# HenryHZY/VL-PET

Hardware: AMD Instinct MI355X
Metric: multitask samples/sec (BART-base, r=96) (higher is better)
Workload: dtype bf16

## Files before the change

### include/vlpet_hip.h

```cpp
#ifndef VLPET_HIP_H
#define VLPET_HIP_H
#include <stddef.h>
#include <stdint.h>

#ifdef __cplusplus
extern "C" {
#endif

#define VLPET_F32 0
#define VLPET_BF16 1

#define VLPET_E_SHAPE (-1)
#define VLPET_E_RANK (-2)
#define VLPET_E_ALIGN (-3)
#define VLPET_E_WORKSPACE (-4)
#define VLPET_E_NULL (-5)
#define VLPET_E_DTYPE (-6)
#define VLPET_E_ALIAS (-7)

#define VLPET_GATE_NONE 0
#define VLPET_GATE_MUL 1
#define VLPET_GATE_ADD 2

typedef void* vlpet_stream_t;

int vlpet_version(void);
const char* vlpet_error_string(int code);

int vlpet_rank_tiles(int r);

size_t vlpet_packed_bytes(int tiles, int d, int io_dtype);
int vlpet_pack_pair(const void* const* wd_heads, const void* const* bd_heads, int n_heads,
                    const void* wu, const void* bu, int r, int d, int tiles,
// ... 203 lines not shown
int vlpet_act_dropout_fwd(const void* x, void* out, uint8_t* keep_out, int64_t n, int act, float p, uint64_t seed,
                          int io_dtype, vlpet_stream_t stream);
int vlpet_act_dropout_bwd(const void* dy, const void* x, void* dx, int64_t n, int act, float p, uint64_t seed,
                          int io_dtype, vlpet_stream_t stream);
int vlpet_concat_dropout_fwd(const void* a, const void* v, void* x, int64_t B, int La, int Lv, int d, float p, uint64_t seed,
                             int io_dtype, vlpet_stream_t stream);
int vlpet_concat_dropout_bwd(const void* dx, void* da, void* dv, int64_t B, int La, int Lv, int d, float p, uint64_t seed,
                             int io_dtype, vlpet_stream_t stream);

int vlpet_ce_loss_fwd(const void* logits, const int64_t* labels, float* loss, float* lse, int64_t N, int V, int ld,
                      int io_dtype, vlpet_stream_t stream);
int vlpet_ce_loss_bwd(const void* logits, const int64_t* labels, const float* lse, const float* dloss, void* dlogits,
                      int64_t N, int V, int ld, int io_dtype, vlpet_stream_t stream);
int vlpet_ce_loss_fwd_checked(const void* logits, const int64_t* labels, float* loss, float* lse, unsigned int* bad_count,
                              int64_t N, int V, int ld, int io_dtype, vlpet_stream_t stream);

#define VLPET_ATTN_MAX_LEN 128
int vlpet_attn_fwd(const void* q, const void* k, const void* v, const uint8_t* key_mask, void* o, float* lse, uint8_t* keep_out,
                   int B, int H, int Lq, int Lk, int causal, float scale, float p, uint64_t seed, vlpet_stream_t stream);
int vlpet_attn_bwd(const void* q, const void* k, const void* v, const void* o, const void* dout, const float* lse,
                   const uint8_t* key_mask, void* dq, void* dk, void* dv, int B, int H, int Lq, int Lk, int causal,
                   float scale, float p, uint64_t seed, vlpet_stream_t stream);
int vlpet_attn_fwd_ld(const void* q, const void* k, const void* v, const uint8_t* key_mask, void* o, float* lse, uint8_t* keep_out,
                      int B, int H, int Lq, int Lk, int ld_q, int ld_kv, int causal, float scale, float p, uint64_t seed,
                      vlpet_stream_t stream);
int vlpet_attn_bwd_ld(const void* q, const void* k, const void* v, const void* o, const void* dout, const float* lse,
                      const uint8_t* key_mask, void* dq, void* dk, void* dv, int B, int H, int Lq, int Lk, int ld_q, int ld_kv,
                      int causal, float scale, float p, uint64_t seed, vlpet_stream_t stream);
int vlpet_attn_fwd_bias(const void* q, const void* k, const void* v, const uint8_t* key_mask, const float* bias, void* o,
                        float* lse, uint8_t* keep_out, int B, int H, int Lq, int Lk, int ld_q, int ld_kv, int causal,
// ... 112 lines not shown
```

### vl-pet_amd/_lib.py

```python
from __future__ import annotations

import ctypes
import os
from ctypes import c_char_p, c_float, c_int, c_int64, c_size_t, c_uint64, c_void_p

_HERE = os.path.dirname(os.path.abspath(__file__))
LIB_PATH = os.environ.get("VLPET_LIB") or os.path.join(_HERE, "lib", "libvlpet_hip.so")

VLPET_F32 = 0
VLPET_BF16 = 1
GATE_NONE, GATE_MUL, GATE_ADD = 0, 1, 2

_lib = None

SIGNATURES = {
    "vlpet_version": (c_int, []),
    "vlpet_error_string": (c_char_p, [c_int]),
    "vlpet_rank_tiles": (c_int, [c_int]),
    "vlpet_packed_bytes": (c_size_t, [c_int, c_int, c_int]),
    "vlpet_pack_pair": (c_int, [c_void_p, c_void_p, c_int, c_void_p, c_void_p, c_int, c_int, c_int, c_int, c_int,
                                c_void_p, c_void_p]),
    "vlpet_pack_pairs": (c_int, [c_int, c_void_p, c_void_p, c_int, c_void_p, c_void_p, c_int, c_int, c_int, c_int, c_int,
                                 c_void_p, c_void_p]),
    "vlpet_adapter_gate_fwd": (c_int, [c_void_p, c_void_p, c_void_p, c_void_p, c_void_p, c_int64, c_int, c_int,
# ... 99 lines not shown
    "vlpet_attn_bwd": (c_int, [c_void_p] * 10 + [c_int] * 5 + [c_float, c_float, c_uint64, c_void_p]),
    "vlpet_attn_fwd_ld": (c_int, [c_void_p] * 7 + [c_int] * 7 + [c_float, c_float, c_uint64, c_void_p]),
    "vlpet_attn_bwd_ld": (c_int, [c_void_p] * 10 + [c_int] * 7 + [c_float, c_float, c_uint64, c_void_p]),
    "vlpet_attn_fwd_bias": (c_int, [c_void_p] * 8 + [c_int] * 7 + [c_float, c_float, c_uint64, c_void_p]),
    "vlpet_attn_bwd_bias": (c_int, [c_void_p] * 12 + [c_int] * 7 + [c_float, c_float, c_uint64, c_void_p]),
    "vlpet_concat_dropout_fwd": (c_int, [c_void_p] * 3 + [c_int64, c_int, c_int, c_int, c_float, c_uint64, c_int, c_void_p]),
    "vlpet_concat_dropout_bwd": (c_int, [c_void_p] * 3 + [c_int64, c_int, c_int, c_int, c_float, c_uint64, c_int, c_void_p]),
    "vlpet_attn_fwd_kv": (c_int, [c_void_p] * 8 + [c_int] * 8 + [c_float, c_float, c_uint64, c_void_p]),
    "vlpet_attn_bwd_kv": (c_int, [c_void_p] * 12 + [c_int] * 8 + [c_float, c_float, c_uint64, c_void_p]),
    "vlpet_attn_long_fwd": (c_int, [c_void_p] * 7 + [c_int] * 8 + [c_float, c_void_p]),
    "vlpet_attn_long_fwd_train": (c_int, [c_void_p] * 8 + [c_int] * 8 + [c_float, c_float, c_uint64, c_void_p]),
    "vlpet_attn_long_bwd": (c_int, [c_void_p] * 12 + [c_int] * 8 + [c_float, c_float, c_uint64, c_void_p, c_void_p]),
    "vlpet_ce_loss_fwd": (c_int, [c_void_p] * 4 + [c_int64, c_int, c_int, c_int, c_void_p]),
    "vlpet_ce_loss_fwd_checked": (c_int, [c_void_p] * 5 + [c_int64, c_int, c_int, c_int, c_void_p]),
    "vlpet_ce_loss_bwd": (c_int, [c_void_p] * 5 + [c_int64, c_int, c_int, c_int, c_void_p]),
    "vlpet_act_dropout_fwd": (c_int, [c_void_p] * 3 + [c_int64, c_int, c_float, c_uint64, c_int, c_void_p]),
    "vlpet_act_dropout_bwd": (c_int, [c_void_p] * 3 + [c_int64, c_int, c_float, c_uint64, c_int, c_void_p]),
    "vlpet_attn_decode": (c_int, [c_void_p, c_int64, c_void_p, c_void_p, c_int64, c_int64, c_int64, c_int64, c_void_p, c_void_p,
                                  c_int64, c_int, c_void_p, c_int64, c_void_p, c_int64, c_void_p, c_int64, c_int, c_int, c_int,
                                  c_int, c_float, c_int, c_void_p]),
    "vlpet_greedy_pick": (c_int, [c_void_p, c_int64, c_int, c_void_p, c_int64, c_int, c_void_p, c_void_p, c_int, c_int, c_int,
                                  c_int, c_int, c_int, c_void_p]),
    "vlpet_attn_decode_beam": (c_int, [c_void_p, c_int64, c_void_p, c_void_p, c_int64, c_int64, c_int64, c_int64, c_void_p,
                                       c_void_p, c_int64, c_int, c_void_p, c_int64, c_void_p, c_int64, c_void_p, c_int64, c_int,
                                       c_int, c_int, c_int, c_float, c_int, c_void_p, c_int64, c_int, c_void_p]),
    "vlpet_beam_rows": (c_int, [c_void_p, c_int64, c_int, c_void_p, c_int64, c_int, c_int, c_int, c_int, c_int, c_int, c_int, c_int,
                                c_void_p, c_void_p, c_void_p, c_int, c_void_p]),
    "vlpet_beam_advance": (c_int, [c_void_p, c_void_p, c_void_p, c_int, c_int, c_int, c_int, c_void_p, c_void_p, c_void_p, c_int64,
                                   c_void_p, c_void_p, c_int64, c_void_p, c_void_p, c_void_p, c_void_p, c_int64, c_void_p,
                                   c_void_p, c_void_p, c_int, c_int, c_int, c_float, c_int, c_void_p]),
# ... 47 lines not shown
```

### vl-pet_amd/csrc/api.hip

```cpp
#include <atomic>
#include "../../include/vlpet_hip.h"
#include "common.h"
#include "kernels.h"
#include <cmath>
#include <stdlib.h>
#include <stdio.h>
#include <vector>

#define VLPET_VERSION 670
#define VLPET_VERSION_R3 300
#define VLPET_VERSION_R2 221

static inline bool aligned16(const void* p) { return (reinterpret_cast<uintptr_t>(p) & 15) == 0; }
static inline size_t align256(size_t v) { return (v + 255) / 256 * 256; }
static inline int herr(hipError_t e) { return e == hipSuccess ? 0 : (int)e; }

extern "C" int vlpet_version(void) { return VLPET_VERSION; }
extern "C" int vlpet_debug_build(void) { return VLPET_IS_DEBUG_BUILD; }

__global__ __launch_bounds__(64) void hold_cus_kernel(unsigned* release, unsigned long long ticks) {
    extern __shared__ __attribute__((aligned(16))) uint8_t hold_smem[];
    typedef __attribute__((address_space(1))) unsigned gu32;
    if (threadIdx.x == 0) {
        hold_smem[0] = 1;
// ... 11 lines not shown
    hipLaunchKernelGGL(hold_cus_kernel, dim3((unsigned)workgroups), dim3(64), (size_t)lds_bytes, (hipStream_t)stream,
                       reinterpret_cast<unsigned*>(release_flag), (unsigned long long)max_ms * 100000ull);
    return herr(hipGetLastError());
}

extern "C" const char* vlpet_error_string(int code) {
    switch (code) {
        case 0: return "success";
        case VLPET_E_SHAPE: return "bad shape (need M > 0, d % 64 == 0, r > 0)";
        case VLPET_E_RANK: return "unsupported bottleneck rank (max 192) or tile count";
        case VLPET_E_ALIGN: return "pointer not 16-byte aligned";
        case VLPET_E_WORKSPACE: return "workspace too small";
        case VLPET_E_NULL: return "required pointer is NULL";
        case VLPET_E_DTYPE: return "unsupported dtype";
        case VLPET_E_ALIAS: return "output overlaps an input";
        default: return code > 0 ? hipGetErrorString((hipError_t)code) : "unknown error";
    }
}

extern "C" int vlpet_rank_tiles(int r) {
    if (r <= 0) return VLPET_E_SHAPE;
    if (r <= 32) return 1;
    if (r <= 96) return 3;
    if (r <= 192) return 6;
    return VLPET_E_RANK;
}

static inline bool tiles_ok(int t) { return t == 1 || t == 3 || t == 6; }
static inline bool dtype_ok(int t) { return t == VLPET_F32 || t == VLPET_BF16; }

// ... 1306 lines not shown
    return vlpet_ce_loss_fwd_checked(logits, labels, loss, lse, nullptr, N, V, ld, io_dtype, stream);
}

extern "C" int vlpet_ce_loss_bwd(const void* logits, const int64_t* labels, const float* lse, const float* dloss, void* dlogits,
                                 int64_t N, int V, int ld, int io_dtype, vlpet_stream_t stream) {
    int rc = ce_common(N, V, ld, io_dtype);
    if (rc) return rc;
    if (!logits || !labels || !lse || !dloss || !dlogits) return VLPET_E_NULL;
    if (!aligned16(logits) || !aligned16(dlogits)) return VLPET_E_ALIGN;
    CeArgs a{};
    a.logits = logits; a.labels = labels; a.loss = nullptr; a.lse = const_cast<float*>(lse); a.dloss = dloss; a.dlogits = dlogits;
    a.N = N; a.V = V; a.ld = ld;
    return herr(launch_ce(a, true, io_dtype == VLPET_F32, (hipStream_t)stream));
}

static int act_common(int64_t n, int act, float p, int io_dtype) {
    if (n <= 0 || (n & 7) != 0) return VLPET_E_SHAPE;
    if (act != VLPET_ACT_GELU && act != VLPET_ACT_GELU_NEW && act != VLPET_ACT_RELU) return VLPET_E_SHAPE;
    if (!(p >= 0.0f && p < 1.0f)) return VLPET_E_SHAPE;
    if (io_dtype != VLPET_F32 && io_dtype != VLPET_BF16) return VLPET_E_DTYPE;
    return 0;
}

extern "C" int vlpet_act_dropout_fwd(const void* x, void* out, uint8_t* keep_out, int64_t n, int act, float p, uint64_t seed,
                                     int io_dtype, vlpet_stream_t stream) {
    int rc = act_common(n, act, p, io_dtype);
    if (rc) return rc;
    if (!x || !out) return VLPET_E_NULL;
    if (!aligned16(x) || !aligned16(out)) return VLPET_E_ALIGN;
    ActDropArgs a{};
// ... 261 lines not shown
```

### vl-pet_amd/csrc/celoss.hip

```cpp
#include "common.h"
#include "kernels.h"
#include "vec8.h"

#define CE_THREADS 256

__device__ __forceinline__ float wave_max(float v) {
#pragma unroll
    for (int o = 32; o > 0; o >>= 1) v = fmaxf(v, __shfl_xor(v, o));
    return v;
}
__device__ __forceinline__ float wave_sum(float v) {
#pragma unroll
    for (int o = 32; o > 0; o >>= 1) v += __shfl_xor(v, o);
    return v;
}

template <typename IO>
__global__ __launch_bounds__(CE_THREADS) void ce_fwd_kernel(CeArgs a) {
    __shared__ float sm[CE_THREADS / 64], ss[CE_THREADS / 64];
    const int64_t n = blockIdx.x;
    const int64_t lab = a.labels[n];
    if (lab < 0 || lab >= a.V) {
        if (threadIdx.x == 0) {
            a.loss[n] = 0.f; a.lse[n] = 0.f;
            if (a.bad != nullptr && lab != -100) atomicAdd(a.bad, 1u);
        }
        return;
    }
    const IO* row = reinterpret_cast<const IO*>(a.logits) + n * (int64_t)a.ld;
    const int groups = (a.V + 7) >> 3;
    float m = -INFINITY, s = 0.f;
    for (int g = threadIdx.x; g < groups; g += CE_THREADS) {
        Vec8<IO> x;
        x.load(row, g);
        float v[8], cm = -INFINITY;
#pragma unroll
        for (int j = 0; j < 8; ++j) {
            v[j] = (8 * g + j < a.V) ? x.get(j) : -INFINITY;
            cm = fmaxf(cm, v[j]);
        }
        const float mn = fmaxf(m, cm);
        float acc = 0.f;
#pragma unroll
        for (int j = 0; j < 8; ++j) acc += __expf(v[j] - mn);
        s = s * __expf(m - mn) + acc;
        m = mn;
    }
    const int wave = threadIdx.x >> 6, lane = threadIdx.x & 63;
    const float wm = wave_max(m);
    const float wsum = wave_sum(m == -INFINITY ? 0.f : s * __expf(m - wm));
    if (lane == 0) { sm[wave] = wm; ss[wave] = wsum; }
    __syncthreads();
    if (threadIdx.x == 0) {
        float M = sm[0];
#pragma unroll
        for (int w = 1; w < CE_THREADS / 64; ++w) M = fmaxf(M, sm[w]);
        float S = 0.f;
#pragma unroll
        for (int w = 0; w < CE_THREADS / 64; ++w) S += ss[w] * __expf(sm[w] - M);
        const float lse = M + __logf(S);
        a.lse[n] = lse;
        a.loss[n] = lse - (float)row[lab];
    }
}

template <typename IO>
__global__ __launch_bounds__(CE_THREADS) void ce_bwd_kernel(CeArgs a) {
    const int64_t n = blockIdx.x;
    const int64_t lab = a.labels[n];
    const bool live = lab >= 0 && lab < a.V;
    const float g = live ? a.dloss[n] : 0.f;
    const IO* row = reinterpret_cast<const IO*>(a.logits) + n * (int64_t)a.ld;
    IO* out = reinterpret_cast<IO*>(a.dlogits) + n * (int64_t)a.ld;
    const int groups = a.ld >> 3;
    if (g == 0.f) {
// ... 6 lines not shown
    const float lse = a.lse[n];
    for (int gi = threadIdx.x; gi < groups; gi += CE_THREADS) {
        Vec8<IO> x, o;
        x.load(row, gi);
#pragma unroll
        for (int j = 0; j < 8; ++j) {
            const int v = 8 * gi + j;
            float p = v < a.V ? __expf(x.get(j) - lse) : 0.f;
            if (v == (int)lab) p -= 1.0f;
            o.set(j, g * p);
        }
        o.store(out, gi);
    }
}

hipError_t launch_ce(const CeArgs& a, bool bwd, int io_fp32, hipStream_t stream) {
    if (a.N <= 0) return hipSuccess;
    const dim3 grid((unsigned)a.N), blk(CE_THREADS);
    if (bwd) {
        if (io_fp32) hipLaunchKernelGGL(ce_bwd_kernel<float>, grid, blk, 0, stream, a);
        else hipLaunchKernelGGL(ce_bwd_kernel<__bf16>, grid, blk, 0, stream, a);
    } else {
        if (io_fp32) hipLaunchKernelGGL(ce_fwd_kernel<float>, grid, blk, 0, stream, a);
        else hipLaunchKernelGGL(ce_fwd_kernel<__bf16>, grid, blk, 0, stream, a);
    }
    return hipGetLastError();
}
```

### vl-pet_amd/csrc/kernels.h

```cpp
#pragma once
#include <cstdlib>
#include <hip/hip_runtime.h>
#include <stdint.h>
#include "rng.h"
#include "tuning.h"

#define VLPET_MAX_HEADS 16

struct PackArgs {
    const void* wd[VLPET_MAX_HEADS];
    const void* bd[VLPET_MAX_HEADS];
    const void* wu;
    const void* bu;
    int n_heads, rows_per_head;
    int r, d, RT;
    int src_bf16;
    int n_packs;
    uint8_t* out;
};
hipError_t launch_pack_pair(const PackArgs& a, int NS, hipStream_t stream);
#define VLPET_PACK_BATCH 8
struct PackBatch { PackArgs p[VLPET_PACK_BATCH]; int n; };
hipError_t launch_pack_pairs(const PackBatch& b, int NS, hipStream_t stream);

// ... 341 lines not shown
hipError_t launch_cat_dropout(const void* a, const void* v, void* x, int64_t B, int La, int Lv, int d, uint32_t thr, float keep_scale,
                              uint64_t seed, const uint64_t* seed_ctr, bool bwd, int io_fp32, hipStream_t stream);

struct CeArgs {
    const void* logits;
    const int64_t* labels;
    float* loss;
    float* lse;
    const float* dloss;
    void* dlogits;
    int64_t N;
    int V, ld;
    unsigned int* bad;
};
hipError_t launch_ce(const CeArgs& a, bool bwd, int io_fp32, hipStream_t stream);

struct AttnArgs {
    const __bf16* q; const __bf16* k; const __bf16* v;
    __bf16* o;
    float* lse;
    const __bf16* dout;
    __bf16* dq; __bf16* dk; __bf16* dv;
    const uint8_t* key_mask;
    const float* bias;
    const float* bias_t;
    uint8_t* keep_out;
    int B, H, Lq, Lk, causal;
    int ld_q, ld_kv;
    int ld_v;
    float scale;
// ... 49 lines not shown
```

### vl-pet_amd/functional.py

```python
from __future__ import annotations

import ctypes
from typing import Optional, Sequence

import torch
import torch.nn.functional as F

from . import _lib

GATE_NONE, GATE_MUL, GATE_ADD = _lib.GATE_NONE, _lib.GATE_MUL, _lib.GATE_ADD


class KernelTimer:

    def __init__(self, names=None):
        self.records = []
        self.names = None if names is None else frozenset(names)

    def wants(self, name):
        return self.names is None or name in self.names

    def bracket(self, name, rows, fn):
        e0 = torch.cuda.Event(enable_timing=True)
        e1 = torch.cuda.Event(enable_timing=True)
# ... 42 lines not shown
    if not _PENDING_REDUCES:
        return 0
    jobs, n = list(_PENDING_REDUCES), len(_PENDING_REDUCES)
    _PENDING_REDUCES.clear()
    vp, ip = ctypes.c_void_p * n, ctypes.c_int * n
    rc = _lib.load().vlpet_reduce_batch(vp(*[j[0].data_ptr() for j in jobs]), vp(*[_ptr(j[3]) for j in jobs]), vp(*[_ptr(j[4]) for j in jobs]),
                                        ip(*[j[1] for j in jobs]), ip(*[j[2] for j in jobs]), n, _stream())
    _lib.check(rc, "vlpet_reduce_batch")
    return n


def _timed(name, rows, fn):
    if TIMER is None or not TIMER.wants(name):
        return fn()
    return TIMER.bracket(name, rows, fn)


def _io_dtype(t: torch.Tensor) -> int:
    if t.dtype == torch.bfloat16:
        return _lib.VLPET_BF16
    if t.dtype == torch.float32:
        return _lib.VLPET_F32
    raise RuntimeError(f"vl-pet_amd: unsupported activation dtype {t.dtype} (bf16 or fp32)")


def _param_dtype(t: torch.Tensor) -> int:
    return _io_dtype(t)


def _stream() -> int:
# ... 777 lines not shown
```

### vl-pet_amd/host/bart.py

```python
from __future__ import annotations

import copy
import math
from types import SimpleNamespace

import torch
import torch.nn as nn
import torch.nn.functional as F

from .. import attention as A
from .. import decode as D
from .. import functional as VF
from .. import adapter_tail as AT
from ..adapters import AdapterController
from ..encoder_pet import apply_pet, build_pet, has_pet
from ..lora import LoRALinearController, LoraConfig
from ..visual import Downsample, LowRankVisualEmbedding, VisualEmbedding
from .common import (COMPACTER_DEFAULTS, check_sequential_adapter_flags, derived_weights, eval_no_grad, fused_adapter_tail,
                     install_shared_phm_rule, is_key_mask, make_adapter_config, sequential_adapters, shift_right, unpack_vis_inputs,
                     value_parallel_adapter)

TASKS = ["vqa", "gqa", "nlvr", "caption"]


# ... 122 lines not shown
EAGER_FFN_ACT = False


def lm_loss(h, weight, labels, bias=None):
    if EAGER_LM_LOSS:
        logits = F.linear(h, weight.to(h.dtype))
        if bias is not None:
            logits = logits + bias.to(h.dtype)
        loss = F.cross_entropy(logits.float().view(-1, logits.shape[-1]), labels.view(-1), ignore_index=-100, reduction="none")
        return loss.view(labels.shape), logits
    from ..lmloss import lm_head_loss
    return lm_head_loss(h, weight, labels, bias)


EAGER_LM_LOSS = False


def _linear(mod: nn.Linear, x):
    w, b = mod.weight, mod.bias
    if w.dtype != x.dtype:
        w = w.to(x.dtype)
    if FUSE_BIAS_GRAD and b is not None and b.requires_grad:
        if VF.linear_train_bias_ok(x, w, b):
            return VF.linear_train_bias(x, w, b)
    if b is not None and b.dtype != x.dtype:
        b = b.to(x.dtype)
    return F.linear(x, w, b)


def _sdpa_ctx():
    import contextlib
# ... 371 lines not shown
        elif isinstance(m, nn.Embedding):
            m.weight.data.normal_(0.0, std)
            if m.padding_idx is not None:
                m.weight.data[m.padding_idx].zero_()
        if isinstance(m, LoRALinearController):
            for t in m.tasks:
                nn.init.zeros_(m.lora_Bs[t])

    def _logits_bias(self):
        b = self.final_logits_bias
        key = (b.data_ptr(), b._version, VF.FROZEN_EPOCH)
        if getattr(self, "_bias_key", None) != key:
            self._bias_key, self._bias_nonzero = key, bool(b.any())
        return b if self._bias_nonzero else None

    def forward(self, input_ids, vis_inputs, labels, task, attention_mask=None, no_padding=False):
        cfg = self.config
        enc, mask = self.model.encoder(input_ids, vis_inputs, attention_mask, task, no_padding)
        dec_in = shift_tokens_right(labels, cfg.pad_token_id, cfg.decoder_start_token_id)
        h = self.model.decoder(dec_in, enc, mask, task)
        return lm_loss(h, self.model.shared.weight, labels, self._logits_bias())

    def generate(self, input_ids, vis_inputs, task, attention_mask=None, max_length=20, min_length=0, no_repeat_ngram_size=0,
                 eos_token_id=None, pad_token_id=None, no_padding=False, num_beams=1, length_penalty=1.0, early_stopping=False,
                 graph=False):
        from ..lmloss import _padded_head
        cfg = self.config
        eos = getattr(cfg, "eos_token_id", 2) if eos_token_id is None else eos_token_id
        pad = cfg.pad_token_id if pad_token_id is None else pad_token_id
        with eval_no_grad(self):
            enc, mask = self.model.encoder(input_ids, vis_inputs, attention_mask, task, no_padding)
            key_mask = None if mask is None else mask[:, 0, 0, :].contiguous()
            dec = self.model.decoder
            state = dec.init_cache(enc, key_mask, task, max_length, num_beams=int(num_beams))
            V = self.model.shared.weight.shape[0]
# ... 18 lines not shown
```

### vl-pet_amd/host/t5.py

```python
from __future__ import annotations

import copy
import math
from types import SimpleNamespace

import torch
import torch.nn as nn
import torch.nn.functional as F

from .. import attention as A
from .. import decode as D
from .. import functional as VF
from .. import adapter_tail as AT
from ..adapters import AdapterController
from ..encoder_pet import apply_pet, build_pet, has_pet
from ..visual import Downsample, T5LayerNorm, VisualEmbedding
from .bart import TASKS, _linear
from .common import (COMPACTER_DEFAULTS, check_sequential_adapter_flags, derived_weights, eval_no_grad, fused_adapter_tail,
                     install_shared_phm_rule, make_adapter_config, sequential_adapters, shift_right, unpack_vis_inputs,
                     value_parallel_adapter)


FUSE_RESIDUAL_GRAD = True

# ... 59 lines not shown

def _tail_or_adapter(ctl, task, hidden, y, p, training, link, layer):
    if ctl is not None:
        return _adapter_then_tail(ctl, task, hidden, y, p, training, link, layer)
    return _tail_linked(hidden, y, p, training, link, layer=layer)


def ffn_activation(x, act, p, training):
    from ..act import act_dropout
    return act_dropout(x, act, p, training)


def lm_loss(h, weight, labels, bias=None):
    from ..lmloss import lm_head_loss
    return lm_head_loss(h, weight, labels, bias)


def sublayer_tail(residual, h, norm, p, training, link=None):
    from ..tail import sublayer_tail as _hip_tail
    return _hip_tail(residual, h, norm, p, training, link=link)


_HIP_SUBLAYER_TAIL = sublayer_tail


def _wire_next_norms(blocks, final_norm):
    subs = [m for b in blocks for m in b.layer]
    for i, m in enumerate(subs):
        object.__setattr__(m, "_next_norm", ((subs[i + 1].layer_norm if i + 1 < len(subs) else final_norm),))

# ... 421 lines not shown
        if isinstance(m, T5LayerNorm):
            m.weight.data.fill_(f * 1.0)
        elif isinstance(m, VLT5):
            m.shared.weight.data.normal_(0.0, f * 1.0)
        elif isinstance(m, T5DenseReluDense):
            m.wi.weight.data.normal_(0.0, f * d ** -0.5)
            m.wo.weight.data.normal_(0.0, f * self.config.d_ff ** -0.5)
        elif isinstance(m, T5Attention):
            m.q.weight.data.normal_(0.0, f * (d * dkv) ** -0.5)
            m.k.weight.data.normal_(0.0, f * d ** -0.5)
            m.v.weight.data.normal_(0.0, f * d ** -0.5)
            m.o.weight.data.normal_(0.0, f * (H * dkv) ** -0.5)
            if m.has_relative_attention_bias:
                m.relative_attention_bias.weight.data.normal_(0.0, f * d ** -0.5)

    def forward(self, input_ids, vis_inputs, labels, task, attention_mask=None, no_padding=False):
        cfg = self.config
        enc, keep = self.encoder(input_ids, vis_inputs, attention_mask, task)
        dec_in = shift_right(labels, cfg.pad_token_id, cfg.decoder_start_token_id)
        h = self.decoder(dec_in, enc, keep, task) * (cfg.d_model ** -0.5)
        return lm_loss(h, self.shared.weight, labels)

    def generate(self, input_ids, vis_inputs, task, attention_mask=None, max_length=20, min_length=0, no_repeat_ngram_size=0,
                 eos_token_id=None, pad_token_id=None, no_padding=False, num_beams=1, length_penalty=1.0, early_stopping=False,
                 graph=False):
        from ..lmloss import _padded_head
        cfg = self.config
        eos = getattr(cfg, "eos_token_id", 1) if eos_token_id is None else eos_token_id
        pad = cfg.pad_token_id if pad_token_id is None else pad_token_id
        with eval_no_grad(self):
            enc, keep = self.encoder(input_ids, vis_inputs, attention_mask, task)
            state = self.decoder.init_cache(enc, (keep > 0.5).contiguous(), task, max_length, num_beams=int(num_beams))
            V = self.shared.weight.shape[0]
            head = _padded_head(self.shared.weight, enc.dtype)
            scale = cfg.d_model ** -0.5
# ... 11 lines not shown
```

### vl-pet_amd/lmloss.py

```python
from __future__ import annotations

from typing import Optional, Tuple

import torch
import torch.nn.functional as F

from . import _lib
from .functional import _io_dtype, _need_cuda, _stream, _timed


def _frozen_epoch():
    from . import functional as _VF
    return _VF.FROZEN_EPOCH


class _CeFn(torch.autograd.Function):
    @staticmethod
    def forward(ctx, logits, labels, V):
        lib = _lib.load()
        _need_cuda(logits, labels)
        N, ld = logits.shape
        io = _io_dtype(logits)
        lab = labels.contiguous()
        if lab.dtype != torch.int64:
# ... 10 lines not shown

    @staticmethod
    def backward(ctx, dloss):
        lib = _lib.load()
        logits, lab, lse = ctx.saved_tensors
        V, io = ctx.cfg
        N, ld = logits.shape
        g = dloss.contiguous().float()
        dlogits = torch.empty_like(logits)
        rc = _timed("ce_bwd", N, lambda: lib.vlpet_ce_loss_bwd(logits.data_ptr(), lab.data_ptr(), lse.data_ptr(), g.data_ptr(),
                                                               dlogits.data_ptr(), N, V, ld, io, _stream()))
        _lib.check(rc, "vlpet_ce_loss_bwd")
        return dlogits, None, None


def cross_entropy_rows(logits: torch.Tensor, labels: torch.Tensor, V: Optional[int] = None) -> torch.Tensor:
    if logits.dim() != 2 or not logits.is_contiguous():
        raise RuntimeError("vl-pet_amd: cross_entropy_rows needs contiguous [N, ld] logits")
    V = logits.shape[1] if V is None else int(V)
    if logits.shape[1] % 8 != 0:
        raise RuntimeError("vl-pet_amd: logits row stride must be a multiple of 8 (use lm_head_loss, which pads the head)")
    labels = labels.reshape(-1)
    if logits.shape[0] == 0:
        return logits.new_zeros(0, dtype=torch.float32) + 0.0 * logits.float().sum()
    _check_labels_once(labels, V)
    return _CeFn.apply(logits, labels, V)


CHECK_LABELS = "once"
_CHECKED = set()
# ... 30 lines not shown
    Vp = (V + 7) // 8 * 8
    if weight.requires_grad:
        w = weight.to(dtype)
        return w if Vp == V else torch.cat([w, w.new_zeros(Vp - V, d)], 0)
    key = (weight.data_ptr(), weight._version, dtype, tuple(weight.shape), _frozen_epoch())
    hit = getattr(weight, "_vlpet_padded_head", None)
    if hit is not None and hit[0] == key:
        return hit[1]
    with torch.no_grad():
        wp = torch.zeros(Vp, d, dtype=dtype, device=weight.device)
        wp[:V].copy_(weight)
    weight._vlpet_padded_head = (key, wp)
    return wp


def lm_head_loss(h: torch.Tensor, weight: torch.Tensor, labels: torch.Tensor,
                 bias: Optional[torch.Tensor] = None) -> Tuple[torch.Tensor, torch.Tensor]:
    V = weight.shape[0]
    wp = _padded_head(weight, h.dtype)
    logits = F.linear(h, wp)
    if bias is not None and bool(bias.any()):
        logits = logits + F.pad(bias.to(h.dtype).reshape(-1), (0, wp.shape[0] - V))
    flat = logits.reshape(-1, wp.shape[0])
    loss = cross_entropy_rows(flat, labels, V)
    return loss.view(labels.shape), logits[..., :V]
```

### vl-pet_amd/train.py

```python
from __future__ import annotations

import collections
import math
import os
import random
from typing import Dict, List, Optional, Sequence

import torch
import torch.distributed as dist
import torch.nn as nn

TASK_BATCH = {"vqa": lambda b: b, "gqa": lambda b: int(b * 100 / 60), "nlvr": lambda b: int(b * 20 / 60),
              "caption": lambda b: int(b * 50 / 60),
              "tvqa": lambda b: b, "how2qa": lambda b: b, "tvc": lambda b: b, "yc2c": lambda b: b}
TEXT_LEN = {"vqa": 20, "gqa": 20, "nlvr": 20, "caption": 40, "tvqa": 600, "how2qa": 600, "tvc": 600, "yc2c": 600}
TARGET_LEN = {"vqa": 5, "gqa": 5, "nlvr": 2, "caption": 20, "tvqa": 3, "how2qa": 3, "tvc": 20, "yc2c": 20}
VIDEO_TASKS = ("tvqa", "how2qa", "tvc", "yc2c")
VIDEO_FRAMES = 64


def trainable_names(model: nn.Module, config) -> List[str]:
    names = []
    for n, p in model.named_parameters():
        p.requires_grad = False
# ... 518 lines not shown
        for k in sorted(batch):
            v = batch[k]
            if torch.is_tensor(v):
                out.append((k, None, v))
            elif isinstance(v, (tuple, list)):
                out += [(k, i, t) for i, t in enumerate(v) if torch.is_tensor(t)]
        return out

    @staticmethod
    def _signature(batch):
        return (batch["task"], bool(batch.get("no_padding", False)),
                tuple((k, i, tuple(t.shape), t.dtype, tuple(t.stride())) for k, i, t in Trainer._leaves(batch)))

    def _fwd_bwd(self, batch) -> torch.Tensor:
        per_token, _ = self.model(batch["input_ids"], batch["vis_inputs"], batch["labels"], batch["task"],
                                  attention_mask=batch.get("attention_mask"), no_padding=bool(batch.get("no_padding", False)))
        loss = task_loss(per_token, batch["labels"], batch.get("scores"), batch["task"])
        if self.flat.flat.is_cuda:
            from . import functional as VF
            alone = (not self.flat.dp) or self.flat.defer
            VF.DEFER_REDUCES = DEFER_PARAM_REDUCES and alone
            fin_was = VF.K1_BWD_FINALIZE_LAUNCH
            VF.K1_BWD_FINALIZE_LAUNCH = bool(fin_was or VF.WGRAD_STREAM is not None or not alone)
            try:
                loss.backward()
                VF.flush_reduces()
            finally:
                VF.K1_BWD_FINALIZE_LAUNCH = fin_was
                VF.DEFER_REDUCES = False
                VF.discard_pending()
        else:
# ... 122 lines not shown
```

Baseline: 29990.

## Fuse LM-head cross-entropy forward and gradient into one pass, drop kept logits

Adds a kernel that keeps a whole logits row in registers, computes the log-sum-exp and loss, and writes softmax-minus-onehot into the logits buffer in the same pass. The separate backward CE read of logits disappears, and the per-row upstream gradient is applied after the dh matmul with a small row-scale kernel. Training no longer keeps the logits tensor, so G overwrites it in place. The cost is heavy register use (25 Vec8 per thread), which may lower occupancy, and the gradient is always computed during forward.

After: 30140 (median of 6 runs). No clear change (+0.5%).

```diff
diff --git a/include/vlpet_hip.h b/include/vlpet_hip.h
--- a/include/vlpet_hip.h
+++ b/include/vlpet_hip.h
@@ -17,6 +17,7 @@
 #define VLPET_E_NULL (-5)
 #define VLPET_E_DTYPE (-6)
 #define VLPET_E_ALIAS (-7)
+#define VLPET_E_DECLINED (-8)
 
 #define VLPET_GATE_NONE 0
 #define VLPET_GATE_MUL 1
@@ -250,6 +251,10 @@
                       int64_t N, int V, int ld, int io_dtype, vlpet_stream_t stream);
 int vlpet_ce_loss_fwd_checked(const void* logits, const int64_t* labels, float* loss, float* lse, unsigned int* bad_count,
                               int64_t N, int V, int ld, int io_dtype, vlpet_stream_t stream);
+#define VLPET_CE_ONEPASS_MAX_LD 51200
+int vlpet_ce_loss_fwd_grad(const void* logits, const int64_t* labels, float* loss, float* lse, unsigned int* bad_count, void* grad_out,
+                           int64_t N, int V, int ld, int io_dtype, vlpet_stream_t stream);
+int vlpet_row_scale(const void* in, const float* s, void* out, int64_t N, int d, int io_dtype, vlpet_stream_t stream);
 
 #define VLPET_ATTN_MAX_LEN 128
 int vlpet_attn_fwd(const void* q, const void* k, const void* v, const uint8_t* key_mask, void* o, float* lse, uint8_t* keep_out,
diff --git a/vl-pet_amd/_lib.py b/vl-pet_amd/_lib.py
--- a/vl-pet_amd/_lib.py
+++ b/vl-pet_amd/_lib.py
@@ -137,6 +137,8 @@
     "vlpet_ce_loss_fwd": (c_int, [c_void_p] * 4 + [c_int64, c_int, c_int, c_int, c_void_p]),
     "vlpet_ce_loss_fwd_checked": (c_int, [c_void_p] * 5 + [c_int64, c_int, c_int, c_int, c_void_p]),
     "vlpet_ce_loss_bwd": (c_int, [c_void_p] * 5 + [c_int64, c_int, c_int, c_int, c_void_p]),
+    "vlpet_ce_loss_fwd_grad": (c_int, [c_void_p] * 6 + [c_int64, c_int, c_int, c_int, c_void_p]),
+    "vlpet_row_scale": (c_int, [c_void_p] * 3 + [c_int64, c_int, c_int, c_void_p]),
     "vlpet_act_dropout_fwd": (c_int, [c_void_p] * 3 + [c_int64, c_int, c_float, c_uint64, c_int, c_void_p]),
     "vlpet_act_dropout_bwd": (c_int, [c_void_p] * 3 + [c_int64, c_int, c_float, c_uint64, c_int, c_void_p]),
     "vlpet_attn_decode": (c_int, [c_void_p, c_int64, c_void_p, c_void_p, c_int64, c_int64, c_int64, c_int64, c_void_p, c_void_p,
diff --git a/vl-pet_amd/csrc/api.hip b/vl-pet_amd/csrc/api.hip
--- a/vl-pet_amd/csrc/api.hip
+++ b/vl-pet_amd/csrc/api.hip
@@ -7,7 +7,7 @@
 #include <stdio.h>
 #include <vector>
 
-#define VLPET_VERSION 670
+#define VLPET_VERSION 680
 #define VLPET_VERSION_R3 300
 #define VLPET_VERSION_R2 221
 
@@ -49,6 +49,7 @@
         case VLPET_E_NULL: return "required pointer is NULL";
         case VLPET_E_DTYPE: return "unsupported dtype";
         case VLPET_E_ALIAS: return "output overlaps an input";
+        case VLPET_E_DECLINED: return "this form does not take the shape (use the general entry points)";
         default: return code > 0 ? hipGetErrorString((hipError_t)code) : "unknown error";
     }
 }
@@ -1385,6 +1386,34 @@
     return herr(launch_ce(a, true, io_dtype == VLPET_F32, (hipStream_t)stream));
 }
 
+static_assert(VLPET_CE_ONEPASS_MAX_LD == CE_ONEPASS_MAX_LD, "the header's limit is the kernel's");
+extern "C" int vlpet_ce_loss_fwd_grad(const void* logits, const int64_t* labels, float* loss, float* lse, unsigned int* bad_count,
+                                      void* grad_out, int64_t N, int V, int ld, int io_dtype, vlpet_stream_t stream) {
+    int rc = ce_common(N, V, ld, io_dtype);
+    if (rc) return rc;
+    if (!logits || !labels || !loss || !lse || !grad_out) return VLPET_E_NULL;
+    if (!aligned16(logits) || !aligned16(grad_out)) return VLPET_E_ALIGN;
+    if (grad_out != logits) {
+        const size_t bytes = (size_t)N * (size_t)ld * (io_dtype == VLPET_F32 ? 4 : 2);
+        const uintptr_t x = reinterpret_cast<uintptr_t>(logits), g = reinterpret_cast<uintptr_t>(grad_out);
+        if (x < g + bytes && g < x + bytes) return VLPET_E_ALIAS;
+    }
+    if (ld > VLPET_CE_ONEPASS_MAX_LD) return VLPET_E_DECLINED;
+    CeArgs a{};
+    a.logits = logits; a.labels = labels; a.loss = loss; a.lse = lse; a.dloss = nullptr; a.dlogits = grad_out;
+    a.N = N; a.V = V; a.ld = ld; a.bad = bad_count;
+    return herr(launch_ce_loss_grad(a, io_dtype == VLPET_F32, (hipStream_t)stream));
+}
+
+extern "C" int vlpet_row_scale(const void* in, const float* s, void* out, int64_t N, int d, int io_dtype, vlpet_stream_t stream) {
+    if (N <= 0 || d <= 0 || (d & 7) != 0) return VLPET_E_SHAPE;
+    if (io_dtype != VLPET_F32 && io_dtype != VLPET_BF16) return VLPET_E_DTYPE;
+    if (!in || !s || !out) return VLPET_E_NULL;
+    if (!aligned16(in) || !aligned16(out)) return VLPET_E_ALIGN;
+    if (N * (int64_t)(d >> 3) > (int64_t)0x7fffffff * 256) return VLPET_E_SHAPE;
+    return herr(launch_row_scale(in, s, out, N, d, io_dtype == VLPET_F32, (hipStream_t)stream));
+}
+
 static int act_common(int64_t n, int act, float p, int io_dtype) {
     if (n <= 0 || (n & 7) != 0) return VLPET_E_SHAPE;
     if (act != VLPET_ACT_GELU && act != VLPET_ACT_GELU_NEW && act != VLPET_ACT_RELU) return VLPET_E_SHAPE;
diff --git a/vl-pet_amd/csrc/celoss.hip b/vl-pet_amd/csrc/celoss.hip
--- a/vl-pet_amd/csrc/celoss.hip
+++ b/vl-pet_amd/csrc/celoss.hip
@@ -13,6 +13,41 @@
 #pragma unroll
     for (int o = 32; o > 0; o >>= 1) v += __shfl_xor(v, o);
     return v;
+}
+
+template <typename IO>
+__device__ __forceinline__ void ce_fold_group(const Vec8<IO>& x, int g, int V, float& m, float& s) {
+    float v[8], cm = -INFINITY;
+#pragma unroll
+    for (int j = 0; j < 8; ++j) {
+        v[j] = (8 * g + j < V) ? x.get(j) : -INFINITY;
+        cm = fmaxf(cm, v[j]);
+    }
+    const float mn = fmaxf(m, cm);
+    float acc = 0.f;
+#pragma unroll
+    for (int j = 0; j < 8; ++j) acc += __expf(v[j] - mn);
+    s = s * __expf(m - mn) + acc;
+    m = mn;
+}
+
+__device__ __forceinline__ float ce_row_lse(float m, float s, float* sm, float* ss) {
+    const int wave = threadIdx.x >> 6, lane = threadIdx.x & 63;
+    const float wm = wave_max(m);
+    const float wsum = wave_sum(m == -INFINITY ? 0.f : s * __expf(m - wm));
+    if (lane == 0) { sm[wave] = wm; ss[wave] = wsum; }
+    __syncthreads();
+    float lse = 0.f;
+    if (threadIdx.x == 0) {
+        float M = sm[0];
+#pragma unroll
+        for (int w = 1; w < CE_THREADS / 64; ++w) M = fmaxf(M, sm[w]);
+        float S = 0.f;
+#pragma unroll
+        for (int w = 0; w < CE_THREADS / 64; ++w) S += ss[w] * __expf(sm[w] - M);
+        lse = M + __logf(S);
+    }
+    return lse;
 }
 
 template <typename IO>
@@ -33,32 +68,10 @@
     for (int g = threadIdx.x; g < groups; g += CE_THREADS) {
         Vec8<IO> x;
         x.load(row, g);
-        float v[8], cm = -INFINITY;
-#pragma unroll
-        for (int j = 0; j < 8; ++j) {
-            v[j] = (8 * g + j < a.V) ? x.get(j) : -INFINITY;
-            cm = fmaxf(cm, v[j]);
-        }
-        const float mn = fmaxf(m, cm);
-        float acc = 0.f;
-#pragma unroll
-        for (int j = 0; j < 8; ++j) acc += __expf(v[j] - mn);
-        s = s * __expf(m - mn) + acc;
-        m = mn;
-    }
-    const int wave = threadIdx.x >> 6, lane = threadIdx.x & 63;
-    const float wm = wave_max(m);
-    const float wsum = wave_sum(m == -INFINITY ? 0.f : s * __expf(m - wm));
-    if (lane == 0) { sm[wave] = wm; ss[wave] = wsum; }
-    __syncthreads();
+        ce_fold_group(x, g, a.V, m, s);
+    }
+    const float lse = ce_row_lse(m, s, sm, ss);
     if (threadIdx.x == 0) {
-        float M = sm[0];
-#pragma unroll
-        for (int w = 1; w < CE_THREADS / 64; ++w) M = fmaxf(M, sm[w]);
-        float S = 0.f;
-#pragma unroll
-        for (int w = 0; w < CE_THREADS / 64; ++w) S += ss[w] * __expf(sm[w] - M);
-        const float lse = M + __logf(S);
         a.lse[n] = lse;
         a.loss[n] = lse - (float)row[lab];
     }
@@ -95,6 +108,85 @@
     }
 }
 
+#define CE_ROW_GROUPS 25
+static_assert(CE_ONEPASS_MAX_LD == 8 * CE_THREADS * CE_ROW_GROUPS, "the limit in kernels.h is what a workgroup holds");
+
+__device__ __forceinline__ void ce_pin(Vec8<__bf16>& x) {
+    f32x4 t = __builtin_bit_cast(f32x4, x.v);
+    asm volatile("" : "+v"(t));
+    x.v = __builtin_bit_cast(bf16x8, t);
+}
+__device__ __forceinline__ void ce_pin(Vec8<float>& x) { asm volatile("" : "+v"(x.a), "+v"(x.b)); }
+
+template <typename IO>
+__global__ __launch_bounds__(CE_THREADS) void ce_loss_grad_kernel(CeArgs a) {
+    __shared__ float sm[CE_THREADS / 64], ss[CE_THREADS / 64];
+    __shared__ float row_lse;
+    const int64_t n = blockIdx.x;
+    const int64_t lab = a.labels[n];
+    IO* out = reinterpret_cast<IO*>(a.dlogits) + n * (int64_t)a.ld;
+    const int all_groups = a.ld >> 3;
+    if (lab < 0 || lab >= a.V) {
+        if (threadIdx.x == 0) {
+            a.loss[n] = 0.f; a.lse[n] = 0.f;
+            if (a.bad != nullptr && lab != -100) atomicAdd(a.bad, 1u);
+        }
+        Vec8<IO> z;
+#pragma unroll
+        for (int j = 0; j < 8; ++j) z.set(j, 0.f);
+        for (int g = threadIdx.x; g < all_groups; g += CE_THREADS) z.store(out, g);
+        return;
+    }
+    const IO* row = reinterpret_cast<const IO*>(a.logits) + n * (int64_t)a.ld;
+    const int groups = (a.V + 7) >> 3;
+    const int t = threadIdx.x;
+    Vec8<IO> x[CE_ROW_GROUPS];
+#pragma unroll
+    for (int i = 0; i < CE_ROW_GROUPS; ++i)
+        if (t < groups - i * CE_THREADS) x[i].load(row + i * (CE_THREADS * 8), t);
+    float m = -INFINITY, s = 0.f;
+#pragma unroll
+    for (int i = 0; i < CE_ROW_GROUPS; ++i)
+        if (t < groups - i * CE_THREADS) ce_fold_group(x[i], t, a.V - i * (CE_THREADS * 8), m, s);
+#pragma unroll
+    for (int i = 0; i < CE_ROW_GROUPS; ++i) ce_pin(x[i]);
+    const float lse0 = ce_row_lse(m, s, sm, ss);
+    if (threadIdx.x == 0) {
+        a.lse[n] = lse0;
+        a.loss[n] = lse0 - (float)row[lab];
+        row_lse = lse0;
+    }
+    __syncthreads();
+    const float lse = row_lse;
+#pragma unroll
+    for (int i = 0; i < CE_ROW_GROUPS; ++i) {
+        if (t < all_groups - i * CE_THREADS) {
+            const int Vi = a.V - i * (CE_THREADS * 8), labi = (int)lab - i * (CE_THREADS * 8);
+            Vec8<IO> o;
+#pragma unroll
+            for (int j = 0; j < 8; ++j) {
+                const int v = 8 * t + j;
+                float p = v < Vi ? __expf(x[i].get(j) - lse) : 0.f;
+                if (v == labi) p -= 1.0f;
+                o.set(j, p);
+            }
+            o.store(out + i * (CE_THREADS * 8), t);
+        }
+    }
+}
+
+template <typename IO>
+__global__ __launch_bounds__(CE_THREADS) void row_scale_kernel(const void* in, const float* s, void* out, int64_t groups, int gpr) {
+    const int64_t g = blockIdx.x * (int64_t)CE_THREADS + threadIdx.x;
+    if (g >= groups) return;
+    const float w = s[g / gpr];
+    Vec8<IO> x;
+    x.load(in, g);
+#pragma unroll
+    for (int j = 0; j < 8; ++j) x.set(j, w * x.get(j));
+    x.store(out, g);
+}
+
 hipError_t launch_ce(const CeArgs& a, bool bwd, int io_fp32, hipStream_t stream) {
     if (a.N <= 0) return hipSuccess;
     const dim3 grid((unsigned)a.N), blk(CE_THREADS);
@@ -107,3 +199,20 @@
     }
     return hipGetLastError();
 }
+
+hipError_t launch_ce_loss_grad(const CeArgs& a, int io_fp32, hipStream_t stream) {
+    if (a.N <= 0) return hipSuccess;
+    const dim3 grid((unsigned)a.N), blk(CE_THREADS);
+    if (io_fp32) hipLaunchKernelGGL(ce_loss_grad_kernel<float>, grid, blk, 0, stream, a);
+    else hipLaunchKernelGGL(ce_loss_grad_kernel<__bf16>, grid, blk, 0, stream, a);
+    return hipGetLastError();
+}
+
+hipError_t launch_row_scale(const void* in, const float* s, void* out, int64_t N, int d, int io_fp32, hipStream_t stream) {
+    const int64_t groups = N * (int64_t)(d >> 3);
+    if (groups <= 0) return hipSuccess;
+    const dim3 grid((unsigned)((groups + CE_THREADS - 1) / CE_THREADS)), blk(CE_THREADS);
+    if (io_fp32) hipLaunchKernelGGL(row_scale_kernel<float>, grid, blk, 0, stream, in, s, out, groups, d >> 3);
+    else hipLaunchKernelGGL(row_scale_kernel<__bf16>, grid, blk, 0, stream, in, s, out, groups, d >> 3);
+    return hipGetLastError();
+}
diff --git a/vl-pet_amd/csrc/kernels.h b/vl-pet_amd/csrc/kernels.h
--- a/vl-pet_amd/csrc/kernels.h
+++ b/vl-pet_amd/csrc/kernels.h
@@ -379,6 +379,9 @@
     unsigned int* bad;
 };
 hipError_t launch_ce(const CeArgs& a, bool bwd, int io_fp32, hipStream_t stream);
+#define CE_ONEPASS_MAX_LD 51200
+hipError_t launch_ce_loss_grad(const CeArgs& a, int io_fp32, hipStream_t stream);
+hipError_t launch_row_scale(const void* in, const float* s, void* out, int64_t N, int d, int io_fp32, hipStream_t stream);
 
 struct AttnArgs {
     const __bf16* q; const __bf16* k; const __bf16* v;
diff --git a/vl-pet_amd/functional.py b/vl-pet_amd/functional.py
--- a/vl-pet_amd/functional.py
+++ b/vl-pet_amd/functional.py
@@ -80,6 +80,11 @@
     if TIMER is None or not TIMER.wants(name):
         return fn()
     return TIMER.bracket(name, rows, fn)
+
+
+def _untimed(name):
+    if TIMER is not None and TIMER.wants(name):
+        TIMER.records.pop()
 
 
 def _io_dtype(t: torch.Tensor) -> int:
diff --git a/vl-pet_amd/host/bart.py b/vl-pet_amd/host/bart.py
--- a/vl-pet_amd/host/bart.py
+++ b/vl-pet_amd/host/bart.py
@@ -160,7 +160,7 @@
 
 
 EAGER_LM_LOSS = False
-
+_HIP_LM_LOSS = lm_loss
 
 def _linear(mod: nn.Linear, x):
     w, b = mod.weight, mod.bias
@@ -562,11 +562,14 @@
             self._bias_key, self._bias_nonzero = key, bool(b.any())
         return b if self._bias_nonzero else None
 
-    def forward(self, input_ids, vis_inputs, labels, task, attention_mask=None, no_padding=False):
+    def forward(self, input_ids, vis_inputs, labels, task, attention_mask=None, no_padding=False, keep_logits=True):
         cfg = self.config
         enc, mask = self.model.encoder(input_ids, vis_inputs, attention_mask, task, no_padding)
         dec_in = shift_tokens_right(labels, cfg.pad_token_id, cfg.decoder_start_token_id)
         h = self.model.decoder(dec_in, enc, mask, task)
+        if not keep_logits and lm_loss is _HIP_LM_LOSS and not EAGER_LM_LOSS:
+            from ..lmloss import lm_head_loss
+            return lm_head_loss(h, self.model.shared.weight, labels, self._logits_bias(), keep_logits=False)
         return lm_loss(h, self.model.shared.weight, labels, self._logits_bias())
 
     def generate(self, input_ids, vis_inputs, task, attention_mask=None, max_length=20, min_length=0, no_repeat_ngram_size=0,
diff --git a/vl-pet_amd/host/t5.py b/vl-pet_amd/host/t5.py
--- a/vl-pet_amd/host/t5.py
+++ b/vl-pet_amd/host/t5.py
@@ -97,6 +97,9 @@
 def lm_loss(h, weight, labels, bias=None):
     from ..lmloss import lm_head_loss
     return lm_head_loss(h, weight, labels, bias)
+
+
+_HIP_LM_LOSS = lm_loss
 
 
 def sublayer_tail(residual, h, norm, p, training, link=None):
@@ -548,11 +551,14 @@
             if m.has_relative_attention_bias:
                 m.relative_attention_bias.weight.data.normal_(0.0, f * d ** -0.5)
 
-    def forward(self, input_ids, vis_inputs, labels, task, attention_mask=None, no_padding=False):
+    def forward(self, input_ids, vis_inputs, labels, task, attention_mask=None, no_padding=False, keep_logits=True):
         cfg = self.config
         enc, keep = self.encoder(input_ids, vis_inputs, attention_mask, task)
         dec_in = shift_right(labels, cfg.pad_token_id, cfg.decoder_start_token_id)
         h = self.decoder(dec_in, enc, keep, task) * (cfg.d_model ** -0.5)
+        if not keep_logits and lm_loss is _HIP_LM_LOSS:
+            from ..lmloss import lm_head_loss
+            return lm_head_loss(h, self.shared.weight, labels, None, keep_logits=False)
         return lm_loss(h, self.shared.weight, labels)
 
     def generate(self, input_ids, vis_inputs, task, attention_mask=None, max_length=20, min_length=0, no_repeat_ngram_size=0,
diff --git a/vl-pet_amd/lmloss.py b/vl-pet_amd/lmloss.py
--- a/vl-pet_amd/lmloss.py
+++ b/vl-pet_amd/lmloss.py
@@ -6,7 +6,7 @@
 import torch.nn.functional as F
 
 from . import _lib
-from .functional import _io_dtype, _need_cuda, _stream, _timed
+from .functional import _io_dtype, _need_cuda, _stream, _timed, _untimed
 
 
 def _frozen_epoch():
@@ -48,6 +48,80 @@
         return dlogits, None, None
 
 
+ONE_PASS_LOSS = True
+E_DECLINED = -8
+
+
+def row_scale(x: torch.Tensor, s: torch.Tensor, out: Optional[torch.Tensor] = None) -> torch.Tensor:
+    _need_cuda(x, s, out)
+    if x.dim() != 2 or not x.is_contiguous() or s.dtype != torch.float32 or not s.is_contiguous() or s.numel() != x.shape[0]:
+        raise RuntimeError("vl-pet_amd: row_scale needs contiguous x [N, d] and fp32 s [N]")
+    if out is None:
+        out = torch.empty_like(x)
+    elif out.shape != x.shape or out.dtype != x.dtype or not out.is_contiguous():
+        raise RuntimeError("vl-pet_amd: row_scale output must match its input")
+    N, d = x.shape
+    if N:
+        _lib.check(_lib.load().vlpet_row_scale(x.data_ptr(), s.data_ptr(), out.data_ptr(), N, d, _io_dtype(x), _stream()), "vlpet_row_scale")
+    return out
+
+
+class _HeadLossFn(torch.autograd.Function):
+
+    @staticmethod
+    def forward(ctx, h, wp, labels, V, bias_row, keep_logits):
+        lib = _lib.load()
+        _need_cuda(h, wp, labels)
+        logits = F.linear(h, wp)
+        if bias_row is not None:
+            logits += bias_row
+        N, ld = logits.shape
+        io = _io_dtype(logits)
+        lab = labels.contiguous()
+        if lab.dtype != torch.int64:
+            lab = lab.long()
+        loss = torch.empty(N, dtype=torch.float32, device=logits.device)
+        lse = torch.empty(N, dtype=torch.float32, device=logits.device)
+        bad = _bad_counter(logits.device)
+        G = torch.empty_like(logits) if keep_logits else logits
+        rc = _timed("ce_bwd", N, lambda: lib.vlpet_ce_loss_fwd_grad(logits.data_ptr(), lab.data_ptr(), loss.data_ptr(), lse.data_ptr(),
+                                                                    bad.data_ptr(), G.data_ptr(), N, V, ld, io, _stream()))
+        ctx.declined = rc == E_DECLINED
+        ctx.cfg = (V, io)
+        ctx.set_materialize_grads(False)
+        if ctx.declined:
+            _untimed("ce_bwd")
+            rc = _timed("ce_fwd", N, lambda: lib.vlpet_ce_loss_fwd_checked(logits.data_ptr(), lab.data_ptr(), loss.data_ptr(), lse.data_ptr(),
+                                                                           bad.data_ptr(), N, V, ld, io, _stream()))
+            _lib.check(rc, "vlpet_ce_loss_fwd_checked")
+            ctx.save_for_backward(logits, wp, lab, lse)
+        else:
+            _lib.check(rc, "vlpet_ce_loss_fwd_grad")
+            ctx.save_for_backward(G, wp)
+        if not keep_logits:
+            return loss, None
+        ctx.mark_non_differentiable(logits)
+        return loss, logits
+
+    @staticmethod
+    def backward(ctx, dloss, _dlogits):
+        if dloss is None:
+            return None, None, None, None, None, None
+        g = dloss.contiguous().float()
+        if ctx.declined:
+            logits, wp, lab, lse = ctx.saved_tensors
+            V, io = ctx.cfg
+            N, ld = logits.shape
+            G = torch.empty_like(logits)
+            rc = _timed("ce_bwd", N, lambda: _lib.load().vlpet_ce_loss_bwd(logits.data_ptr(), lab.data_ptr(), lse.data_ptr(), g.data_ptr(),
+                                                                           G.data_ptr(), N, V, ld, io, _stream()))
+            _lib.check(rc, "vlpet_ce_loss_bwd")
+            return G.mm(wp), None, None, None, None, None
+        G, wp = ctx.saved_tensors
+        dh = G.mm(wp)
+        return row_scale(dh, g, out=dh), None, None, None, None, None
+
+
 def cross_entropy_rows(logits: torch.Tensor, labels: torch.Tensor, V: Optional[int] = None) -> torch.Tensor:
     if logits.dim() != 2 or not logits.is_contiguous():
         raise RuntimeError("vl-pet_amd: cross_entropy_rows needs contiguous [N, ld] logits")
@@ -108,13 +182,33 @@
     return wp
 
 
+def _bias_row(bias: Optional[torch.Tensor], dtype: torch.dtype, Vp: int) -> Optional[torch.Tensor]:
+    if bias is None:
+        return None
+    key = (bias.data_ptr(), bias._version, dtype, Vp, _frozen_epoch())
+    hit = getattr(bias, "_vlpet_bias_row", None)
+    if hit is None or hit[0] != key:
+        with torch.no_grad():
+            row = F.pad(bias.to(dtype).reshape(-1), (0, Vp - bias.numel())) if bool(bias.any()) else None
+        hit = bias._vlpet_bias_row = (key, row)
+    return hit[1]
+
+
 def lm_head_loss(h: torch.Tensor, weight: torch.Tensor, labels: torch.Tensor,
-                 bias: Optional[torch.Tensor] = None) -> Tuple[torch.Tensor, torch.Tensor]:
+                 bias: Optional[torch.Tensor] = None, keep_logits: bool = True) -> Tuple[torch.Tensor, Optional[torch.Tensor]]:
     V = weight.shape[0]
     wp = _padded_head(weight, h.dtype)
+    Vp = wp.shape[0]
+    row = _bias_row(bias, h.dtype, Vp)
+    if (ONE_PASS_LOSS and torch.is_grad_enabled() and h.requires_grad and not weight.requires_grad
+            and (bias is None or not bias.requires_grad) and h.numel() > 0):
+        flat_labels = labels.reshape(-1)
+        _check_labels_once(flat_labels, V)
+        loss, logits = _HeadLossFn.apply(h.reshape(-1, h.shape[-1]), wp, flat_labels, V, row, keep_logits)
+        return loss.view(labels.shape), (logits.view(*h.shape[:-1], Vp)[..., :V] if keep_logits else None)
     logits = F.linear(h, wp)
-    if bias is not None and bool(bias.any()):
-        logits = logits + F.pad(bias.to(h.dtype).reshape(-1), (0, wp.shape[0] - V))
-    flat = logits.reshape(-1, wp.shape[0])
+    if row is not None:
+        logits = logits + row
+    flat = logits.reshape(-1, Vp)
     loss = cross_entropy_rows(flat, labels, V)
-    return loss.view(labels.shape), logits[..., :V]
+    return loss.view(labels.shape), (logits[..., :V] if keep_logits else None)
diff --git a/vl-pet_amd/train.py b/vl-pet_amd/train.py
--- a/vl-pet_amd/train.py
+++ b/vl-pet_amd/train.py
@@ -556,7 +556,8 @@
 
     def _fwd_bwd(self, batch) -> torch.Tensor:
         per_token, _ = self.model(batch["input_ids"], batch["vis_inputs"], batch["labels"], batch["task"],
-                                  attention_mask=batch.get("attention_mask"), no_padding=bool(batch.get("no_padding", False)))
+                                  attention_mask=batch.get("attention_mask"), no_padding=bool(batch.get("no_padding", False)),
+                                  keep_logits=False)
         loss = task_loss(per_token, batch["labels"], batch.get("scores"), batch["task"])
         if self.flat.flat.is_cuda:
             from . import functional as VF
```
